# LAPKB/pharmsol

Hardware: AMD Instinct MI355X
Metric: subject_event_steps_per_sec (higher is better)
Workload: dtype f64; 1 GPU; C3: two_compartments analytical, 100000 subjects/GPU x 1000 support points, 8 events/subject; subjects_per_gpu=100000, support_points=1000, steps_per_pass=800000000, kernel=pmx_analytical_classed, status_bytes_written=True, prediction_buffer=best of 8 plain allocations, rows padded to 1008 doubles (pmx_recommended_ld), row_pitch_doubles=1008

## Files before the change

### pharmsol_amd/csrc/pmx_classed_ll.hip

```cpp
#include "pmx_lanes.hpp"

namespace pmx {

namespace {

#ifdef PMX_LL_STAMPS
__device__ uint64_t g_ll_stamps[5];
#endif
template <int G>
struct ObsRequest;
template <>
struct ObsRequest<8> {
  typedef u32x16 V;
};
template <>
struct ObsRequest<4> {
  typedef u32x8 V;
};

#ifndef PMX_LL_WAVES
#define PMX_LL_WAVES 3
#endif
template <int KID, bool CENS>
__global__ __launch_bounds__(kBlock, (LaneModel<KID>::NS <= 2) ? PMX_LL_WAVES : 2) void pmx_analytical_classed_ll(
    DevModel m, DevOps ops, DevClassPlan cp, const double* __restrict__ theta, int64_t P, int32_t n_ptiles,
    uint8_t* __restrict__ status) {
  using LM = LaneModel<KID>;
  constexpr int NS = LM::NS;
  constexpr int G = ClassBatch<KID>::G;
  using Req = ObsRequest<G>;
  const auto [ptile, cblock, n_cblocks] = classed_block(n_ptiles);
  const int64_t c_end = cp.n_chunks_exact;
  if (cblock >= c_end) return;
  const uint32_t lane = threadIdx.x & 63u;
  const int64_t p = static_cast<int64_t>(ptile) * kBlock + threadIdx.x;
  const bool lane_ok = p < P;
  const int64_t pc = lane_ok ? p : (P - 1);
  const double* __restrict__ th = theta + pc * m.nparams;
  const double nanv = __longlong_as_double(0x7ff8000000000000LL);

  typename LM::S::Coef coef;
  double inv_vol0;
  bool lane_good;
  double xinit[NS];
  {
    LM L;
    lane_setup<KID, false>(m, th, L);
    coef = L.coef;
    lane_good = L.ok;
    inv_vol0 = L.ok ? L.inv_vol[0] : nanv;
#pragma unroll
    for (int i = 0; i < NS; ++i) xinit[i] = L.xinit[i];
  }
  const auto chunk_row = as_const(cp.chunk_row);
  const auto val = as_const(cp.val);
  const auto cobs = as_const(cp.cobs);
  (void)chunk_row;
  const int out_state0 = m.out[0].state - m.pm;
  const char* hdr_base = reinterpret_cast<const char*>(cp.chunk_hdr);
  char* const ll_lane = reinterpret_cast<char*>(ops.ll_out + p);
  uint32_t ll_pitch = static_cast<uint32_t>(ops.ll_ld * 8);
  asm volatile("" : "+v"(ll_pitch));

#ifdef PMX_LL_STAMPS
  uint64_t tp[5] = {0, 0, 0, 0, 0};
  const uint64_t t_wave0 = __builtin_amdgcn_s_memtime();
#define PMX_STAMP(i, t_prev)                              \
  {                                                       \
    const uint64_t t_now_ = __builtin_amdgcn_s_memtime(); \
    tp[i] += t_now_ - t_prev;                             \
    t_prev = t_now_;                                      \
  }
#else
#define PMX_STAMP(i, t_prev)
#endif

  u32x16 h_n = sload_here<u32x16>(hdr_base + cblock * 64);
  for (int64_t c = cblock; c < c_end; c += n_cblocks) {
#ifdef PMX_LL_STAMPS
    uint64_t t_ph = __builtin_amdgcn_s_memtime();
#endif
    u32x16 h = h_n;
    asm volatile("" : "+s"(h));
    const int32_t n_live = static_cast<int32_t>(h[0] & 0xffffu);
    const int32_t n_steps = static_cast<int32_t>(h[0] >> 16);
    const int64_t pb = static_cast<int64_t>(h[1]);
    int64_t voff = static_cast<int64_t>(h[2]);
    const int64_t cbase = static_cast<int64_t>(h[3]);
    const uint64_t rate_mask = (static_cast<uint64_t>(h[5]) << 32) | h[4];
    uint64_t fast_mask = ((static_cast<uint64_t>(h[7]) << 32) | h[6]) & ~rate_mask & 0x7fffffffffffffffull;
    int32_t sid_park = 0;
#pragma unroll
    for (int j = 0; j < G; ++j) sid_park = (static_cast<int>(lane) == j) ? static_cast<int32_t>(h[8 + j]) : sid_park;
    int64_t cobs_off = cbase + 2 * G;
    if constexpr (CENS) {
      fast_mask &= static_cast<uint64_t>(__double_as_longlong(cobs[cbase + G + 1]));
    }
    if (cp.zero_status == 1 && status != nullptr) {
      const int zj = static_cast<int>(lane >> 3);
      int64_t zsid = -1;
#pragma unroll
      for (int j = 0; j < G; ++j) zsid = (zj == j && j < n_live) ? static_cast<int64_t>(static_cast<int32_t>(h[8 + j])) : zsid;
      const int64_t zp = static_cast<int64_t>(ptile) * kBlock + (threadIdx.x & ~63u) + 8 * (lane & 7u);
      if (zsid >= 0 && zp < P) *reinterpret_cast<uint64_t*>(status + zsid * P + zp) = 0ull;
    }
    double ll_acc[G], x[G][NS];
#pragma unroll
    for (int j = 0; j < G; ++j) {
      ll_acc[j] = 0.0;
#pragma unroll
      for (int i = 0; i < NS; ++i) x[j][i] = 0.0;
    }
    uint32_t bad = 0;
    double ex[LM::S::NE];
#pragma unroll
    for (int i = 0; i < LM::S::NE; ++i) ex[i] = 0.0;
    int32_t kobs = 0;
    bool csum_in = false;
    const double* recs = cp.prog_rec + 2 * pb;
    int32_t k = 0;
    PMX_STAMP(0, t_ph)
    while (k < n_steps) {
      const uint64_t run_bits = (k < 63) ? (fast_mask >> k) : 0ull;
      if (run_bits & 1ull) {
        int32_t run = __builtin_ctzll(~run_bits);
        if (run > n_steps - k) run = n_steps - k;
        const bool closes = (k + run == n_steps);
        auto fast_run = [&](auto st_c) {
          constexpr int ST = decltype(st_c)::value;
          typename Req::V cs_v;
          if (closes) cs_v = sload_here<typename Req::V>(cp.cobs + cbase);
          uint64_t w_n = sload_here<uint64_t>(recs + 2 * k);
#pragma unroll 1
          for (int32_t i = 0; i < run; ++i) {
            uint64_t w = w_n;
            asm volatile("" : "+s"(w));
            const typename Req::V yc = sload_here<typename Req::V>(cp.cobs + cobs_off);
            const typename Req::V wc = sload_here<typename Req::V>(cp.cobs + cobs_off + G);
            w_n = sload_here<uint64_t>(recs + 2 * (k + i + 1));
            __builtin_amdgcn_sched_barrier(0);
            cobs_off += 2 * G;
            double ov_y[G], ov_w[G];
#pragma unroll
            for (int j = 0; j < G; ++j) {
              ov_y[j] = __longlong_as_double(static_cast<int64_t>((static_cast<uint64_t>(yc[2 * j + 1]) << 32) | yc[2 * j]));
              ov_w[j] = __longlong_as_double(static_cast<int64_t>((static_cast<uint64_t>(wc[2 * j + 1]) << 32) | wc[2 * j]));
            }
            const uint32_t rung = (static_cast<uint32_t>(w) >> kOpRungShift) & kOpRungMask;
            if (rung != 1u) {
#pragma unroll
              for (int e = 0; e < LM::S::NE; ++e) {
                const double bse = ex[e];
                const double sq = bse * bse;
                double r = sq;
                if (rung != 2u) r = sq * ((rung == 3u) ? bse : sq);
                ex[e] = r;
              }
            }
            typename LM::S::Prop pr;
            LM::S::from_exps_f(coef, ex, pr);
#pragma unroll
            for (int j = 0; j < G; ++j) LM::S::apply0(pr, x[j]);
#pragma unroll
            for (int j = 0; j < G; ++j) {
              const double d = fma(-inv_vol0, x[j][ST], ov_y[j]);
              ll_acc[j] = fma(-(d * ov_w[j]), d, ll_acc[j]);
            }
          }
          if (closes) {
#pragma unroll
            for (int j = 0; j < G; ++j)
              ll_acc[j] += __longlong_as_double(static_cast<int64_t>((static_cast<uint64_t>(cs_v[2 * j + 1]) << 32) | cs_v[2 * j]));
          }
        };
        if (out_state0 == 0) fast_run(std::integral_constant<int, 0>{});
        if constexpr (NS > 1) {
          if (out_state0 == 1) fast_run(std::integral_constant<int, 1>{});
        }
        if constexpr (NS > 2) {
          if (out_state0 == 2) fast_run(std::integral_constant<int, 2>{});
        }
        if constexpr (NS > 3) {
          if (out_state0 == 3) fast_run(std::integral_constant<int, 3>{});
        }
        kobs += run;
        voff += static_cast<int64_t>(run) * G;
        k += run;
        csum_in = closes;
        PMX_STAMP(2, t_ph)
        continue;
      }
      const auto rp = as_const(reinterpret_cast<const uint64_t*>(recs)) + 2 * k;
      const uint64_t w = rp[0], dtb = rp[1];
      const uint32_t meta = static_cast<uint32_t>(w);
      const uint32_t kind = meta & kOpKindMask;
      const int io = static_cast<int>((meta >> kOpIoShift) & kOpIoMask);
      const bool has_val = ((rate_mask >> (k < 63 ? k : 63)) & 1ull) != 0ull;
      if (kind == OP_PROP) {
        const uint32_t rung = (meta >> kOpRungShift) & kOpRungMask;
        if (rung == 0u) {
          LM::S::exps(coef, __longlong_as_double(static_cast<int64_t>(dtb)), ex);
        } else if (rung != 1u) {
          ladder_pow<LM::S::NE>(ex, rung);
        }
        typename LM::S::Prop pr;
        LM::S::from_exps_f(coef, ex, pr);
#pragma unroll
        for (int j = 0; j < G; ++j) LM::S::apply0(pr, x[j]);
        if (has_val) {
          LM::S::from_exps_j(coef, ex, pr);
#pragma unroll
          for (int j = 0; j < G; ++j) LM::S::add_j(pr, x[j], val[voff + j]);
        }
      } else if (kind == OP_BOLUS) {
        double f = fa_of(m, th, io);
        asm volatile("s_waitcnt vmcnt(0)" : "+v"(f)::"memory");
#pragma unroll
        for (int j = 0; j < G; ++j) {
          const double a = val[voff + j] * f;
#pragma unroll
          for (int i = 0; i < NS; ++i) x[j][i] += (i == io - m.pm) ? a : 0.0;
        }
      } else if (kind == OP_RESET) {
#pragma unroll
        for (int i = 0; i < NS; ++i) {
          const double xi = io ? xinit[i] : 0.0;
#pragma unroll
          for (int j = 0; j < G; ++j) x[j][i] = xi;
        }
      }
      if ((meta >> kOpObsAfterShift) & 1u) {
        const auto ov = cobs + cobs_off;
        double ov_y[G], ov_w[G];
#pragma unroll
        for (int j = 0; j < G; ++j) {
          ov_y[j] = ov[j];
          ov_w[j] = ov[G + j];
        }
        const int oq = static_cast<int>((meta >> kOpOutShift) & kOpOutMask);
        int out_state = out_state0;
        double inv_vol = inv_vol0;
        if (oq != 0) {
          out_state = m.out[oq].state - m.pm;
          const int vp = m.out_vol_theta[oq];
          double v = 1.0;
          if (vp >= 0) v = th[vp];
          double iv = 1.0 / v;
          asm volatile("" : "+v"(iv));
          inv_vol = lane_good ? iv : nanv;
        }
        auto fold = [&](auto st_c) {
          constexpr int ST = decltype(st_c)::value;
#pragma unroll
          for (int j = 0; j < G; ++j) {
            const int64_t wb = __double_as_longlong(ov_w[j]);
            if (wb != 0) {
              if (CENS && wb < 0) {
                ll_accumulate(as_const(ops.ll_obs) + (chunk_row[c * G + j] + kobs) * 4, x[j][ST] * inv_vol, ll_acc[j]);
              } else {
                const double d = fma(-inv_vol, x[j][ST], ov_y[j]);
                ll_acc[j] = fma(-(d * ov_w[j]), d, ll_acc[j]);
              }
            }
          }
        };
        if (out_state == 0) fold(std::integral_constant<int, 0>{});
        if constexpr (NS > 1) {
          if (out_state == 1) fold(std::integral_constant<int, 1>{});
        }
        if constexpr (NS > 2) {
          if (out_state == 2) fold(std::integral_constant<int, 2>{});
        }
        if constexpr (NS > 3) {
          if (out_state == 3) fold(std::integral_constant<int, 3>{});
        }
        cobs_off += 2 * G;
        ++kobs;
      }
      voff += G;
      ++k;
      PMX_STAMP(1, t_ph)
    }
    {
      const int64_t c_next = (c + n_cblocks < c_end) ? (c + n_cblocks) : c;
      h_n = sload_here<u32x16>(hdr_base + c_next * 64);
      __builtin_amdgcn_sched_barrier(0);
    }
    if (!csum_in) {
      const auto cs = cobs + cbase;
#pragma unroll
      for (int j = 0; j < G; ++j) ll_acc[j] += cs[j];
    }
    double nanacc = 0.0;
#pragma unroll
    for (int j = 0; j < G; ++j) {
      if (j < n_live) {
        const double llj = ll_acc[j];
        nanacc = fma(llj, 0.0, nanacc);
        const uint32_t sidj = static_cast<uint32_t>(__builtin_amdgcn_readlane(sid_park, j));
        double* const dst = reinterpret_cast<double*>(ll_lane + static_cast<uint64_t>(sidj) * ll_pitch);
        if (lane_ok) __builtin_nontemporal_store(llj, dst);
      }
    }
    if (status != nullptr) {
      if (__any((nanacc != nanacc) ? 1 : 0)) {
#pragma unroll
        for (int j = 0; j < G; ++j)
          if (j < n_live && !isfinite(ll_acc[j])) bad |= (1u << j);
      }
      if (cp.zero_status == 2 || __any(((bad != 0u || !lane_good) && lane_ok) ? 1 : 0)) {
        if (cp.zero_status == 1) asm volatile("s_waitcnt vmcnt(0)" ::: "memory");
#pragma unroll
        for (int j = 0; j < G; ++j) {
          if (j < n_live) {
            const uint8_t st = !lane_good ? PMX_PAIR_COMPLEX_ROOTS : (((bad >> j) & 1u) ? PMX_PAIR_NONFINITE : PMX_PAIR_OK);
            if (lane_ok && (st != PMX_PAIR_OK || cp.zero_status == 2))
              status[static_cast<int64_t>(__builtin_amdgcn_readlane(sid_park, j)) * P + p] = st;
          }
        }
      }
    }
    PMX_STAMP(3, t_ph)
  }
#ifdef PMX_LL_STAMPS
  tp[4] = __builtin_amdgcn_s_memtime() - t_wave0;
  if ((threadIdx.x & 63u) == 0u)
    for (int i = 0; i < 5; ++i) atomicAdd(reinterpret_cast<unsigned long long*>(&g_ll_stamps[i]), static_cast<unsigned long long>(tp[i]));
#endif
#undef PMX_STAMP
}


}

hipError_t launch_classed_ll(const LaunchArgs& a, const Route& r) {
  if (r.dyn || r.lag) return hipErrorInvalidValue;
  return with_kid(a.m.kernel, [&](auto kid) {
    return dispatch([&](auto cens) {
      hipLaunchKernelGGL((pmx_analytical_classed_ll<decltype(kid)::value, decltype(cens)::value>), dim3(static_cast<uint32_t>(r.blocks)),
                         dim3(r.threads), 0, static_cast<hipStream_t>(a.stream), a.m, a.ops, a.cls, a.theta, a.P, r.n_ptiles, a.status);
      return hipGetLastError();
    }, r.cens);
  });
}

#ifdef PMX_LL_STAMPS
}
extern "C" int32_t pmx_debug_ll_stamps(uint64_t* out5, int32_t reset) {
  uint64_t z[5] = {0, 0, 0, 0, 0};
  if (hipDeviceSynchronize() != hipSuccess) return 1;
  if (out5 && hipMemcpyFromSymbol(out5, HIP_SYMBOL(pmx::g_ll_stamps), sizeof(z)) != hipSuccess) return 2;
  if (reset && hipMemcpyToSymbol(HIP_SYMBOL(pmx::g_ll_stamps), z, sizeof(z)) != hipSuccess) return 3;
  return 0;
}
namespace pmx {
#endif

}
```

Measured before the change: 939.5 billion subject-event-steps/s.

## Add specialized common-chunk path for tied analytical models with hand-tuned step math

Adds a specialized path for chunks matching the common reset+initial-prop+fast-run pattern in one/two-compartment models. It computes the shared first propagation once per lane and broadcasts it to all subjects, then runs a tight observation loop. It also replaces the generic propagator/ladder math with inline-asm FMA sequences and uses writelane/bpermute for subject id parking. The goal is to cut per-step branching and scalar overhead, at the cost of substantially more code, register pressure and a second path to keep consistent.

```diff
diff --git a/pharmsol_amd/csrc/pmx_classed_ll.hip b/pharmsol_amd/csrc/pmx_classed_ll.hip
--- a/pharmsol_amd/csrc/pmx_classed_ll.hip
+++ b/pharmsol_amd/csrc/pmx_classed_ll.hip
@@ -18,6 +18,122 @@
   typedef u32x8 V;
 };
 
+template <int SID>
+struct LLStep {
+  using S = Structure<SID>;
+  using Coef = typename S::Coef;
+  using Prop = typename S::Prop;
+  static constexpr int NS = S::NS, NE = S::NE;
+  static constexpr bool kTied = (SID == S_ONE || SID == S_ONE_ABS || SID == S_TWO);
+
+  template <bool RUN>
+  __device__ __forceinline__ static void make_f(const Coef& c, const double (&e)[NE], Prop& p) {
+    if constexpr (SID == S_TWO) {
+      const TwoCore& t = c.t;
+      const double de = e[1] - e[0];
+      if constexpr (RUN) {
+        p.p.f00 = fma(t.b11, e[1], t.a11 * e[0]);
+        p.p.f11 = fma(t.b22, e[1], t.a22 * e[0]);
+      } else {
+        p.p.f00 = fma(t.a11, e[0], t.b11 * e[1]);
+        p.p.f11 = fma(t.a22, e[0], t.b22 * e[1]);
+      }
+      p.p.f01 = t.kpc * de;
+      p.p.f10 = t.kcp * de;
+    } else {
+      S::from_exps_f(c, e, p);
+    }
+  }
+  __device__ __forceinline__ static void make_j(const Coef& c, const double (&e)[NE], Prop& p) {
+    if constexpr (SID == S_TWO) {
+      const TwoCore& t = c.t;
+      const double o1 = 1.0 - e[0], o2 = 1.0 - e[1];
+      p.p.j0 = fma(t.i0a, o1, t.i0b * o2);
+      p.p.j1 = fma(t.i1a, o1, t.i1b * o2);
+    } else {
+      S::from_exps_j(c, e, p);
+    }
+  }
+  __device__ __forceinline__ static void apply0(const Prop& p, double (&x)[NS]) {
+    if constexpr (SID == S_ONE) {
+      asm("v_mul_f64 %0, %0, %1" : "+v"(x[0]) : "v"(p.e));
+    } else if constexpr (SID == S_ONE_ABS) {
+      asm("v_mul_f64 %1, %3, %1\n\t"
+          "v_fmac_f64 %1, %0, %4\n\t"
+          "v_mul_f64 %0, %2, %0"
+          : "+v"(x[0]), "+v"(x[1])
+          : "v"(p.ea), "v"(p.ee), "v"(p.g));
+    } else if constexpr (SID == S_TWO) {
+      double t;
+      asm("v_mul_f64 %2, %4, %1\n\t"
+          "v_mul_f64 %1, %6, %1\n\t"
+          "v_fmac_f64 %1, %0, %5\n\t"
+          "v_fma_f64 %0, %0, %3, %2"
+          : "+v"(x[0]), "+v"(x[1]), "=&v"(t)
+          : "v"(p.p.f00), "v"(p.p.f01), "v"(p.p.f10), "v"(p.p.f11));
+    } else {
+      S::apply0(p, x);
+    }
+  }
+  __device__ __forceinline__ static void add_j(const Prop& p, double (&x)[NS], double r) {
+    if constexpr (SID == S_ONE) {
+      x[0] = fma(r, p.j, x[0]);
+    } else if constexpr (SID == S_ONE_ABS) {
+      x[1] = fma(r, p.j, x[1]);
+    } else if constexpr (SID == S_TWO) {
+      x[0] = fma(r, p.p.j0, x[0]);
+      x[1] = fma(r, p.p.j1, x[1]);
+    } else {
+      S::add_j(p, x, r);
+    }
+  }
+  __device__ __forceinline__ static void add_j_to(const Prop& p, const double (&fx)[NS], double r, double (&x)[NS]) {
+#pragma unroll
+    for (int i = 0; i < NS; ++i) x[i] = fx[i];
+    if constexpr (SID == S_ONE) {
+      x[0] = fma(r, p.j, fx[0]);
+    } else if constexpr (SID == S_ONE_ABS) {
+      x[1] = fma(r, p.j, fx[1]);
+    } else if constexpr (SID == S_TWO) {
+      x[0] = fma(r, p.p.j0, fx[0]);
+      x[1] = fma(r, p.p.j1, fx[1]);
+    } else {
+      S::add_j(p, x, r);
+    }
+  }
+  __device__ __forceinline__ static void ladder(double (&e)[NE], uint32_t rung) {
+    asm volatile("" : "+s"(rung));
+    if (rung == 3u) {
+#pragma unroll
+      for (int i = 0; i < NE; ++i) {
+        double sq;
+        asm("v_mul_f64 %1, %0, %0\n\t"
+            "v_mul_f64 %0, %1, %0"
+            : "+v"(e[i]), "=&v"(sq));
+      }
+    }
+    asm volatile("" : "+s"(rung));
+    if ((rung & 1u) == 0u) {
+#pragma unroll
+      for (int i = 0; i < NE; ++i) asm("v_mul_f64 %0, %0, %0" : "+v"(e[i]));
+    }
+    asm volatile("" : "+s"(rung));
+    if (rung == 4u) {
+#pragma unroll
+      for (int i = 0; i < NE; ++i) asm("v_mul_f64 %0, %0, %0" : "+v"(e[i]));
+    }
+  }
+};
+typedef uint32_t u32x4 __attribute__((ext_vector_type(4)));
+
+template <int J, int G>
+__device__ __forceinline__ void park_ids(const u32x16& h, int32_t& v) {
+  if constexpr (J < G) {
+    asm("v_writelane_b32 %0, %1, %2" : "+v"(v) : "s"(h[8 + J]), "n"(J));
+    park_ids<J + 1, G>(h, v);
+  }
+}
+
 #ifndef PMX_LL_WAVES
 #define PMX_LL_WAVES 3
 #endif
@@ -29,10 +145,12 @@
   constexpr int NS = LM::NS;
   constexpr int G = ClassBatch<KID>::G;
   using Req = ObsRequest<G>;
+  using Step = LLStep<kernel_structure(KID)>;
   const auto [ptile, cblock, n_cblocks] = classed_block(n_ptiles);
-  const int64_t c_end = cp.n_chunks_exact;
+  const int64_t c_end = cp.n_chunks_exact, c_step = n_cblocks;
   if (cblock >= c_end) return;
   const uint32_t lane = threadIdx.x & 63u;
+  const int32_t zj4 = static_cast<int32_t>(lane >> 3) * 4;
   const int64_t p = static_cast<int64_t>(ptile) * kBlock + threadIdx.x;
   const bool lane_ok = p < P;
   const int64_t pc = lane_ok ? p : (P - 1);
@@ -90,20 +208,184 @@
     const uint64_t rate_mask = (static_cast<uint64_t>(h[5]) << 32) | h[4];
     uint64_t fast_mask = ((static_cast<uint64_t>(h[7]) << 32) | h[6]) & ~rate_mask & 0x7fffffffffffffffull;
     int32_t sid_park = 0;
-#pragma unroll
-    for (int j = 0; j < G; ++j) sid_park = (static_cast<int>(lane) == j) ? static_cast<int32_t>(h[8 + j]) : sid_park;
-    int64_t cobs_off = cbase + 2 * G;
+    park_ids<0, G>(h, sid_park);
+    const int64_t cobs0 = cbase + 2 * G;
+    uint64_t plain_mask = ~0ull;
     if constexpr (CENS) {
-      fast_mask &= static_cast<uint64_t>(__double_as_longlong(cobs[cbase + G + 1]));
+      plain_mask = static_cast<uint64_t>(__double_as_longlong(cobs[cbase + G + 1]));
+      fast_mask &= plain_mask;
     }
     if (cp.zero_status == 1 && status != nullptr) {
-      const int zj = static_cast<int>(lane >> 3);
-      int64_t zsid = -1;
-#pragma unroll
-      for (int j = 0; j < G; ++j) zsid = (zj == j && j < n_live) ? static_cast<int64_t>(static_cast<int32_t>(h[8 + j])) : zsid;
+      const int32_t zsid = __builtin_amdgcn_ds_bpermute(zj4, sid_park);
       const int64_t zp = static_cast<int64_t>(ptile) * kBlock + (threadIdx.x & ~63u) + 8 * (lane & 7u);
-      if (zsid >= 0 && zp < P) *reinterpret_cast<uint64_t*>(status + zsid * P + zp) = 0ull;
-    }
+      if (zj4 < 4 * n_live && zp < P) *reinterpret_cast<uint64_t*>(status + static_cast<int64_t>(zsid) * P + zp) = 0ull;
+    }
+    const double* recs = cp.prog_rec + 2 * pb;
+    PMX_STAMP(0, t_ph)
+
+    auto finish = [&](double (&ll_acc)[G], bool csum_in) __attribute__((always_inline)) {
+      {
+        const int64_t c_next = (c + c_step < c_end) ? (c + c_step) : c;
+        h_n = sload_here<u32x16>(hdr_base + c_next * 64);
+        __builtin_amdgcn_sched_barrier(0);
+      }
+      if (!csum_in) {
+        const auto cs = cobs + cbase;
+#pragma unroll
+        for (int j = 0; j < G; ++j) ll_acc[j] += cs[j];
+      }
+      uint32_t bad = 0;
+      double nanacc = 0.0;
+#pragma unroll
+      for (int j = 0; j < G; ++j) {
+        if (j < n_live) {
+          const double llj = ll_acc[j];
+          nanacc = fma(llj, 0.0, nanacc);
+          const uint32_t sidj = static_cast<uint32_t>(__builtin_amdgcn_readlane(sid_park, j));
+          double* const dst = reinterpret_cast<double*>(ll_lane + static_cast<uint64_t>(sidj) * ll_pitch);
+          if (lane_ok) __builtin_nontemporal_store(llj, dst);
+        }
+      }
+      if (status != nullptr) {
+        if (__any((nanacc != nanacc) ? 1 : 0)) {
+#pragma unroll
+          for (int j = 0; j < G; ++j)
+            if (j < n_live && !isfinite(ll_acc[j])) bad |= (1u << j);
+        }
+        if (cp.zero_status == 2 || __any(((bad != 0u || !lane_good) && lane_ok) ? 1 : 0)) {
+          if (cp.zero_status == 1) asm volatile("s_waitcnt vmcnt(0)" ::: "memory");
+#pragma unroll
+          for (int j = 0; j < G; ++j) {
+            if (j < n_live) {
+              const uint8_t st = !lane_good ? PMX_PAIR_COMPLEX_ROOTS : (((bad >> j) & 1u) ? PMX_PAIR_NONFINITE : PMX_PAIR_OK);
+              if (lane_ok && (st != PMX_PAIR_OK || cp.zero_status == 2))
+                status[static_cast<int64_t>(__builtin_amdgcn_readlane(sid_park, j)) * P + p] = st;
+            }
+          }
+        }
+      }
+    };
+
+    if constexpr (Step::kTied) {
+      const int32_t rest = n_steps - 2;
+      bool common = rest >= 1 && n_steps <= 63 && ((plain_mask >> 1) & 1ull) != 0ull && out_state0 >= 0 && out_state0 < NS;
+      if (common) {
+        const uint64_t need = ((1ull << rest) - 1ull) << 2;
+        common = (fast_mask & need) == need;
+      }
+      if (common) {
+        const uint32_t m0 = sload_here<uint32_t>(recs);
+        const u32x4 r1 = sload_here<u32x4>(recs + 2);
+        const uint64_t w2 = sload_here<uint64_t>(recs + 4);
+        __builtin_amdgcn_sched_barrier(0);
+        const uint32_t m1 = r1[0];
+        const bool open_ok = (m0 & kOpKindMask) == OP_RESET && ((m0 >> kOpObsAfterShift) & 1u) == 0u && (m1 & kOpKindMask) == OP_PROP &&
+                             ((m1 >> kOpRungShift) & kOpRungMask) == 0u && ((m1 >> kOpObsAfterShift) & 1u) != 0u &&
+                             ((m1 >> kOpOutShift) & kOpOutMask) == 0u && (m1 >> kOpFlushShift) == 0u;
+        if (open_ok) {
+          const typename Req::V rv = sload_here<typename Req::V>(cp.val + voff + G);
+          __builtin_amdgcn_sched_barrier(0);
+          auto common_chunk = [&](auto st_c, double (&ll_acc)[G]) __attribute__((always_inline)) {
+            constexpr int ST = decltype(st_c)::value;
+            const bool init = ((m0 >> kOpIoShift) & kOpIoMask) != 0u;
+            const double dt1 = __longlong_as_double(static_cast<int64_t>((static_cast<uint64_t>(r1[3]) << 32) | r1[2]));
+            double ex[Step::NE];
+            LM::S::exps(coef, dt1, ex);
+            typename LM::S::Prop pr;
+            Step::template make_f<false>(coef, ex, pr);
+            double fx[NS];
+#pragma unroll
+            for (int i = 0; i < NS; ++i) fx[i] = init ? xinit[i] : 0.0;
+            Step::apply0(pr, fx);
+            double x[G][NS];
+            if ((rate_mask >> 1) & 1ull) {
+              Step::make_j(coef, ex, pr);
+#pragma unroll
+              for (int j = 0; j < G; ++j)
+                Step::add_j_to(pr, fx, __longlong_as_double(static_cast<int64_t>((static_cast<uint64_t>(rv[2 * j + 1]) << 32) | rv[2 * j])), x[j]);
+            } else {
+#pragma unroll
+              for (int j = 0; j < G; ++j)
+#pragma unroll
+                for (int i = 0; i < NS; ++i) x[j][i] = fx[i];
+            }
+            const double* co = cp.cobs + cobs0;
+            {
+              const typename Req::V yc = sload_here<typename Req::V>(co);
+              const typename Req::V wc = sload_here<typename Req::V>(co + G);
+              __builtin_amdgcn_sched_barrier(0);
+#pragma unroll
+              for (int j = 0; j < G; ++j) {
+                const uint64_t wb = (static_cast<uint64_t>(wc[2 * j + 1]) << 32) | wc[2 * j];
+                ll_acc[j] = 0.0;
+                if (wb != 0ull) {
+                  asm volatile("");
+                  const double yj = __longlong_as_double(static_cast<int64_t>((static_cast<uint64_t>(yc[2 * j + 1]) << 32) | yc[2 * j]));
+                  const double d = fma(-inv_vol0, x[j][ST], yj);
+                  ll_acc[j] = fma(-(d * __longlong_as_double(static_cast<int64_t>(wb))), d, ll_acc[j]);
+                }
+              }
+            }
+            PMX_STAMP(1, t_ph)
+            auto step = [&](uint64_t w, const typename Req::V& yc, const typename Req::V& wc) __attribute__((always_inline)) {
+              const uint32_t rung = (static_cast<uint32_t>(w) >> kOpRungShift) & kOpRungMask;
+              Step::ladder(ex, rung);
+              Step::template make_f<true>(coef, ex, pr);
+#pragma unroll
+              for (int j = 0; j < G; ++j) Step::apply0(pr, x[j]);
+#pragma unroll
+              for (int j = 0; j < G; ++j) {
+                const double yj = __longlong_as_double(static_cast<int64_t>((static_cast<uint64_t>(yc[2 * j + 1]) << 32) | yc[2 * j]));
+                const double wj = __longlong_as_double(static_cast<int64_t>((static_cast<uint64_t>(wc[2 * j + 1]) << 32) | wc[2 * j]));
+                const double d = fma(-inv_vol0, x[j][ST], yj);
+                ll_acc[j] = fma(-(d * wj), d, ll_acc[j]);
+              }
+            };
+            uint64_t w_n = w2;
+            const double* rn = recs + 6;
+#pragma unroll 1
+            for (int32_t i = 1; i < rest; ++i) {
+              uint64_t w = w_n;
+              asm volatile("" : "+s"(w));
+              co += 2 * G;
+              const typename Req::V yc = sload_here<typename Req::V>(co);
+              const typename Req::V wc = sload_here<typename Req::V>(co + G);
+              w_n = sload_here<uint64_t>(rn);
+              __builtin_amdgcn_sched_barrier(0);
+              rn += 2;
+              step(w, yc, wc);
+            }
+            {
+              uint64_t w = w_n;
+              asm volatile("" : "+s"(w));
+              co += 2 * G;
+              const typename Req::V yc = sload_here<typename Req::V>(co);
+              const typename Req::V wc = sload_here<typename Req::V>(co + G);
+              const typename Req::V cs_v = sload_here<typename Req::V>(cp.cobs + cbase);
+              __builtin_amdgcn_sched_barrier(0);
+              step(w, yc, wc);
+#pragma unroll
+              for (int j = 0; j < G; ++j)
+                ll_acc[j] += __longlong_as_double(static_cast<int64_t>((static_cast<uint64_t>(cs_v[2 * j + 1]) << 32) | cs_v[2 * j]));
+            }
+            PMX_STAMP(2, t_ph)
+          };
+          double ll_acc[G];
+          if constexpr (NS > 1) {
+            if (out_state0 == 0)
+              common_chunk(std::integral_constant<int, 0>{}, ll_acc);
+            else
+              common_chunk(std::integral_constant<int, 1>{}, ll_acc);
+          } else {
+            common_chunk(std::integral_constant<int, 0>{}, ll_acc);
+          }
+          finish(ll_acc, true);
+          PMX_STAMP(3, t_ph)
+          continue;
+        }
+      }
+    }
+    int64_t cobs_off = cobs0;
     double ll_acc[G], x[G][NS];
 #pragma unroll
     for (int j = 0; j < G; ++j) {
@@ -111,15 +393,12 @@
 #pragma unroll
       for (int i = 0; i < NS; ++i) x[j][i] = 0.0;
     }
-    uint32_t bad = 0;
     double ex[LM::S::NE];
 #pragma unroll
     for (int i = 0; i < LM::S::NE; ++i) ex[i] = 0.0;
     int32_t kobs = 0;
     bool csum_in = false;
-    const double* recs = cp.prog_rec + 2 * pb;
     int32_t k = 0;
-    PMX_STAMP(0, t_ph)
     while (k < n_steps) {
       const uint64_t run_bits = (k < 63) ? (fast_mask >> k) : 0ull;
       if (run_bits & 1ull) {
@@ -147,20 +426,11 @@
               ov_w[j] = __longlong_as_double(static_cast<int64_t>((static_cast<uint64_t>(wc[2 * j + 1]) << 32) | wc[2 * j]));
             }
             const uint32_t rung = (static_cast<uint32_t>(w) >> kOpRungShift) & kOpRungMask;
-            if (rung != 1u) {
-#pragma unroll
-              for (int e = 0; e < LM::S::NE; ++e) {
-                const double bse = ex[e];
-                const double sq = bse * bse;
-                double r = sq;
-                if (rung != 2u) r = sq * ((rung == 3u) ? bse : sq);
-                ex[e] = r;
-              }
-            }
+            Step::ladder(ex, rung);
             typename LM::S::Prop pr;
-            LM::S::from_exps_f(coef, ex, pr);
-#pragma unroll
-            for (int j = 0; j < G; ++j) LM::S::apply0(pr, x[j]);
+            Step::template make_f<true>(coef, ex, pr);
+#pragma unroll
+            for (int j = 0; j < G; ++j) Step::apply0(pr, x[j]);
 #pragma unroll
             for (int j = 0; j < G; ++j) {
               const double d = fma(-inv_vol0, x[j][ST], ov_y[j]);
@@ -204,13 +474,13 @@
           ladder_pow<LM::S::NE>(ex, rung);
         }
         typename LM::S::Prop pr;
-        LM::S::from_exps_f(coef, ex, pr);
-#pragma unroll
-        for (int j = 0; j < G; ++j) LM::S::apply0(pr, x[j]);
+        Step::template make_f<false>(coef, ex, pr);
+#pragma unroll
+        for (int j = 0; j < G; ++j) Step::apply0(pr, x[j]);
         if (has_val) {
-          LM::S::from_exps_j(coef, ex, pr);
-#pragma unroll
-          for (int j = 0; j < G; ++j) LM::S::add_j(pr, x[j], val[voff + j]);
+          Step::make_j(coef, ex, pr);
+#pragma unroll
+          for (int j = 0; j < G; ++j) Step::add_j(pr, x[j], val[voff + j]);
         }
       } else if (kind == OP_BOLUS) {
         double f = fa_of(m, th, io);
@@ -281,45 +551,7 @@
       ++k;
       PMX_STAMP(1, t_ph)
     }
-    {
-      const int64_t c_next = (c + n_cblocks < c_end) ? (c + n_cblocks) : c;
-      h_n = sload_here<u32x16>(hdr_base + c_next * 64);
-      __builtin_amdgcn_sched_barrier(0);
-    }
-    if (!csum_in) {
-      const auto cs = cobs + cbase;
-#pragma unroll
-      for (int j = 0; j < G; ++j) ll_acc[j] += cs[j];
-    }
-    double nanacc = 0.0;
-#pragma unroll
-    for (int j = 0; j < G; ++j) {
-      if (j < n_live) {
-        const double llj = ll_acc[j];
-        nanacc = fma(llj, 0.0, nanacc);
-        const uint32_t sidj = static_cast<uint32_t>(__builtin_amdgcn_readlane(sid_park, j));
-        double* const dst = reinterpret_cast<double*>(ll_lane + static_cast<uint64_t>(sidj) * ll_pitch);
-        if (lane_ok) __builtin_nontemporal_store(llj, dst);
-      }
-    }
-    if (status != nullptr) {
-      if (__any((nanacc != nanacc) ? 1 : 0)) {
-#pragma unroll
-        for (int j = 0; j < G; ++j)
-          if (j < n_live && !isfinite(ll_acc[j])) bad |= (1u << j);
-      }
-      if (cp.zero_status == 2 || __any(((bad != 0u || !lane_good) && lane_ok) ? 1 : 0)) {
-        if (cp.zero_status == 1) asm volatile("s_waitcnt vmcnt(0)" ::: "memory");
-#pragma unroll
-        for (int j = 0; j < G; ++j) {
-          if (j < n_live) {
-            const uint8_t st = !lane_good ? PMX_PAIR_COMPLEX_ROOTS : (((bad >> j) & 1u) ? PMX_PAIR_NONFINITE : PMX_PAIR_OK);
-            if (lane_ok && (st != PMX_PAIR_OK || cp.zero_status == 2))
-              status[static_cast<int64_t>(__builtin_amdgcn_readlane(sid_park, j)) * P + p] = st;
-          }
-        }
-      }
-    }
+    finish(ll_acc, csum_in);
     PMX_STAMP(3, t_ph)
   }
 #ifdef PMX_LL_STAMPS
```

Measured after the change: 940.1 billion subject-event-steps/s (median of 2 runs). About the same (+0.1%).
